# awsaf49/vip-cup-2022

Hardware: AMD Instinct MI355X
Metric: images/sec (200x200, full ensemble) (higher is better)
Workload: dtype f16; 1 GPU; ensemble8; precision=fast, distinct_images=5120, global_batch=256, parallelism=image-parallel dp1, one all-gather of scores, member_streams=3

## Files before the change

### include/vipcup_hip.h

```cpp
#ifndef VIPCUP_HIP_H
#define VIPCUP_HIP_H

#include <stddef.h>
#include <stdint.h>

#ifdef __cplusplus
extern "C" {
#endif

typedef enum vip_status {
    VIP_OK = 0,
    VIP_ERR_BAD_ARG = -1,
    VIP_ERR_ALIGNMENT = -2,
    VIP_ERR_UNSUPPORTED = -3,
    VIP_ERR_LAUNCH = -4,
    VIP_ERR_JPEG = -5,
    VIP_ERR_PNG = -6,
    VIP_ERR_WEBP = -7
} vip_status;

enum { VIP_ACT_NONE = 0, VIP_ACT_RELU = 1, VIP_ACT_SILU = 2, VIP_ACT_GELU = 3, VIP_ACT_SIGMOID = 4 };

int vip_version(void);
const char* vip_last_error(void);
// ... 34 lines not shown

int vip_ln_gemm_supported(int M, int K, int N, int act);
int vip_ln_gemm_bias_act_f16(const void* A, const float* ln_gamma, const float* ln_beta, float ln_eps, const void* W,
                             const float* bias, const void* residual, void* C, int M, int N, int K, int lda, int ldw,
                             int ldc, int ldr, int act_pre, int act_post, void* stream);

int vip_gemm_split_f16(const void* A, const void* W, const float* bias, void* C, int M, int N, int K, int lda,
                       int ldw, int act, void* stream);

int vip_gemm_split2_f16(const void* A, const void* W, const float* bias, void* C, int M, int N, int K, int ldw, int act,
                        void* stream);
int vip_gemm_split2_hilo_f16(const void* A, const void* W, const void* W_lo, const float* bias, void* C, int M, int N, int K, int ldw,
                             int act, void* stream);

int vip_mlp_fused_supported(int M, int C, int hidden, int act);
int vip_mlp_fused_plan(int M, int C, int hidden, int act, int* workgroups, int* tile_rows);
int vip_mlp_fused_f16(const void* x, const float* ln_gamma, const float* ln_beta, float ln_eps, const void* w1,
                      const float* b1, const void* w2, const float* b2, const void* residual, void* y, int M, int C,
                      int hidden, int ldx, int ldw1, int ldw2, int ldy, int ldr, int act, void* stream);

int vip_se_gate_f16(const void* x, const void* w1, const float* b1, const void* w2, const float* b2, void* gate,
                    int B, int HW, int C, int ldx, int Cr, int ldw1, int Cout, int ldw2, int act1, int act2,
                    int split, void* stream);
int vip_se_gate_hilo_f16(const void* x, const void* w1, const void* w1_lo, const float* b1, const void* w2, const float* b2, void* gate,
                         int B, int HW, int C, int ldx, int Cr, int ldw1, int Cout, int ldw2, int act1, int act2, int split,
                         void* stream);

int vip_dwconv2d_nhwc_f16(const void* x, const float* w, const float* bias, void* y,
                          int B, int H, int W, int C, int k, int stride, int pt, int pl,
                          int Ho, int Wo, int act, void* stream);

int vip_dwconv2d_pool_parts(int B, int H, int W, int C, int k, int stride, int Ho, int Wo);
long vip_dwconv2d_tile_plan(int B, int H, int W, int C, int k, int stride, int Ho, int Wo, int pooled, int* workgroups, int* geom);
int vip_dwconv2d_pool_nhwc_f16(const void* x, const float* w, const float* bias, void* y, float* partials, int parts,
                               int B, int H, int W, int C, int k, int stride, int pt, int pl, int Ho, int Wo, int act,
                               void* stream);
int vip_se_gate_pooled_f16(const float* partials, int parts, const void* w1, const float* b1, const void* w2,
                           const float* b2, void* gate, int B, int HW, int C, int Cr, int ldw1, int Cout, int ldw2,
                           int act1, int act2, int split, void* stream);

int vip_layernorm_f16(const void* x, const float* gamma, const float* beta, void* y,
                      int rows, int C, float eps, void* stream);

int vip_pool2d_nhwc_f16(const void* x, void* y, int B, int H, int W, int C, int ldx, int ldy,
                        int k, int stride, int pt, int pl, int Ho, int Wo, int mode, void* stream);

int vip_global_avgpool_f16(const void* x, void* y, int B, int HW, int C, int ldx, void* stream);

int vip_global_avgpool_split_f16(const void* x, void* y, int B, int HW, int C, int ldx, void* stream);

int vip_gap_dense_f32(const void* x, const float* W, const float* bias, float* out, int B, int HW, int C,
                      int ldx, int N, void* stream);

int vip_gap_ln_dense_f32(const void* x, const float* gamma, const float* beta, float eps, const float* W, const float* bias,
                         float* out, int B, int HW, int C, int ldx, int N, void* stream);

int vip_scale_add_act_f16(const void* x, const void* scale, const void* residual, void* y,
                          int B, int HW, int C, int act, void* stream);
int vip_scale_add_act2_f16(const void* x, const void* scale, const void* residual, void* y, void* y2,
                           int B, int HW, int C, int act, int act2, void* stream);
int vip_scale_add_act3_f16(const void* x, const void* scale, int scale_planes, const void* residual, void* y, void* y2,
                           int B, int HW, int C, int act, int act2, void* stream);

int vip_mul_f16(const void* a, const void* b, void* y, long rows, int C, int lda, int a_off, int ldb, int b_off,
                int ldy, int y_off, void* stream);

// ... 379 lines not shown
```

### vip-cup-2022_amd/_abi.py

```python
import ctypes as C
import os

import torch

_HERE = os.path.dirname(os.path.abspath(__file__))
LIB_PATH = os.environ.get("VIP_LIB_PATH") or os.path.join(_HERE, "libvipcup_hip.so")

_lib = None


class VipError(RuntimeError):
    pass


class ConvDesc(C.Structure):
    _fields_ = [(n, C.c_int) for n in (
        "B", "H", "W", "Cin", "Cout", "kh", "kw", "sh", "sw", "pt", "pl", "Ho", "Wo", "groups",
        "ldx", "cin_off", "ldy", "cout_off", "ldr", "res_off", "ldw", "act_pre", "act_post")]


class JpegDesc(C.Structure):
    _fields_ = [("width", C.c_int32), ("height", C.c_int32), ("ncomp", C.c_int32),
                ("hsamp", C.c_int32 * 3), ("vsamp", C.c_int32 * 3),
                ("blocks_w", C.c_int32 * 3), ("blocks_h", C.c_int32 * 3),
# ... 27 lines not shown

class Vp8EncParams(C.Structure):
    _fields_ = [("quality", C.c_int32), ("base_q", C.c_int32), ("y1", C.c_int32 * 2), ("y2", C.c_int32 * 2), ("uv", C.c_int32 * 2),
                ("filter_level", C.c_int32), ("flevel", C.c_int32), ("ilevel", C.c_int32), ("hev", C.c_int32), ("i4_bias", C.c_int32),
                ("reserved", C.c_int32), ("y1_inv", C.c_uint32 * 2), ("y2_inv", C.c_uint32 * 2), ("uv_inv", C.c_uint32 * 2)]


_vp, _i, _f, _sz = C.c_void_p, C.c_int, C.c_float, C.c_size_t

SIGNATURES = {
    "vip_version": (_i, []),
    "vip_last_error": (C.c_char_p, []),
    "vip_conv2d_nhwc_f16": (_i, [_vp, _vp, _vp, _vp, _vp, C.POINTER(ConvDesc), _vp]),
    "vip_conv2d_gated_nhwc_f16": (_i, [_vp, _vp, _vp, _vp, _vp, _vp, C.POINTER(ConvDesc), _vp]),
    "vip_conv2d_hilo_nhwc_f16": (_i, [_vp, _vp, _vp, _vp, _vp, _vp, C.POINTER(ConvDesc), _vp]),
    "vip_conv2d_out_gated_nhwc_f16": (_i, [_vp, _vp, _vp, _vp, _vp, _vp, _vp, C.POINTER(ConvDesc), _vp]),
    "vip_conv2d_out_gated_variant": (_i, [C.POINTER(ConvDesc), _i, C.c_char_p, _sz]),
    "vip_conv2d_out_gated2_nhwc_f16": (_i, [_vp, _vp, _vp, _vp, _vp, _vp, _vp, _vp, _i, C.POINTER(ConvDesc), _vp]),
    "vip_conv2d_out_gated2_variant": (_i, [C.POINTER(ConvDesc), _i, _i, C.c_char_p, _sz]),
    "vip_gemm_bias_act_f16": (_i, [_vp, _vp, _vp, _vp, _vp] + [_i] * 9 + [_vp]),
    "vip_ln_gemm_supported": (_i, [_i, _i, _i, _i]),
    "vip_ln_gemm_bias_act_f16": (_i, [_vp, _vp, _vp, _f] + [_vp] * 4 + [_i] * 9 + [_vp]),
    "vip_mlp_fused_supported": (_i, [_i, _i, _i, _i]),
    "vip_mlp_fused_plan": (_i, [_i] * 4 + [C.POINTER(_i)] * 2),
    "vip_mlp_fused_f16": (_i, [_vp, _vp, _vp, _f] + [_vp] * 6 + [_i] * 9 + [_vp]),
    "vip_se_gate_f16": (_i, [_vp] * 6 + [_i] * 11 + [_vp]),
    "vip_se_gate_hilo_f16": (_i, [_vp] * 7 + [_i] * 11 + [_vp]),
    "vip_gemm_split_f16": (_i, [_vp, _vp, _vp, _vp] + [_i] * 6 + [_vp]),
    "vip_gemm_split2_f16": (_i, [_vp, _vp, _vp, _vp] + [_i] * 5 + [_vp]),
    "vip_gemm_split2_hilo_f16": (_i, [_vp, _vp, _vp, _vp, _vp] + [_i] * 5 + [_vp]),
    "vip_dwconv2d_nhwc_f16": (_i, [_vp, _vp, _vp, _vp] + [_i] * 11 + [_vp]),
    "vip_dwconv2d_pool_parts": (_i, [_i] * 8),
    "vip_dwconv2d_tile_plan": (C.c_long, [_i] * 9 + [C.POINTER(_i)] * 2),
    "vip_dwconv2d_pool_nhwc_f16": (_i, [_vp, _vp, _vp, _vp, _vp] + [_i] * 12 + [_vp]),
    "vip_se_gate_pooled_f16": (_i, [_vp, _i] + [_vp] * 5 + [_i] * 10 + [_vp]),
    "vip_layernorm_f16": (_i, [_vp, _vp, _vp, _vp, _i, _i, _f, _vp]),
    "vip_pool2d_nhwc_f16": (_i, [_vp, _vp] + [_i] * 13 + [_vp]),
    "vip_global_avgpool_f16": (_i, [_vp, _vp, _i, _i, _i, _i, _vp]),
    "vip_global_avgpool_split_f16": (_i, [_vp, _vp, _i, _i, _i, _i, _vp]),
    "vip_gap_dense_f32": (_i, [_vp, _vp, _vp, _vp, _i, _i, _i, _i, _i, _vp]),
    "vip_experiments_built": (_i, []),
    "vip_gcvit_attn_block_supported": (_i, [_i, _i, _i]),
    "vip_gcvit_attn_block_f16": (_i, [_vp, _vp, _vp, _vp, _f, _vp, _i, _vp, _vp, _i, _vp, _vp, _vp] + [_i] * 6 + [_f, _vp]),
    "vip_mbconv_expand_dw_supported": (_i, [_i, _i, _i, _i]),
    "vip_mbconv_expand_dw_f16": (_i, [_vp] * 7 + [_i] * 14 + [_vp]),
    "vip_head_prob_f32": (_i, [_vp, _vp, _vp, _i, _i, _vp]),
    "vip_head_act_f32": (_i, [_vp, _vp, _i, _i, _i, _vp]),
    "vip_prob_to_score_f32": (_i, [_vp, _vp, _i, _i, _vp]),
    "vip_ensemble_mean_f32": (_i, [_vp, _vp, _i, _i, C.c_long, _vp]),
    "vip_gap_ln_dense_f32": (_i, [_vp, _vp, _vp, _f, _vp, _vp, _vp, _i, _i, _i, _i, _i, _vp]),
    "vip_scale_add_act_f16": (_i, [_vp, _vp, _vp, _vp, _i, _i, _i, _i, _vp]),
    "vip_scale_add_act2_f16": (_i, [_vp, _vp, _vp, _vp, _vp, _i, _i, _i, _i, _i, _vp]),
    "vip_scale_add_act3_f16": (_i, [_vp, _vp, _i, _vp, _vp, _vp, _i, _i, _i, _i, _i, _vp]),
    "vip_mul_f16": (_i, [_vp, _vp, _vp, C.c_long] + [_i] * 7 + [_vp]),
    "vip_radix_combine_f16": (_i, [_vp, _vp, _vp, _i, _i, _i, _i, _vp]),
    "vip_radix_combine2_f16": (_i, [_vp, _vp, _i, _vp, _i, _i, _i, _i, _vp]),
    "vip_window_attn_fwd_f16": (_i, [_vp, _vp, _vp, _vp] + [_i] * 7 + [_f, _vp]),
    "vip_mhsa_fwd_f16": (_i, [_vp, _vp, _i, _i, _i, _i, _f, _vp]),
    "vip_jpeg_probe_h": (_i, [_vp, _sz, _vp, _vp]),
    "vip_jpeg_entropy_decode_h": (_i, [_vp, _vp, _i, _vp, _vp, _sz, _vp, _i]),
    "vip_jpeg_idct_rgb_u8": (_i, [_vp, _vp, _i, _i, _vp, _vp, _i, _i, _vp]),
    "vip_jpeg_quality_tables_h": (_i, [_i, _vp, _vp]),
    "vip_jpeg_encode_layout_h": (_i, [_i, _i, _i, _i, _vp, _vp]),
    "vip_jpeg_fdct_quant_u8": (_i, [_vp, _vp, _i, _i, _vp, _vp, _i, _i, _vp]),
    "vip_resample_coeffs_h": (_i, [_i, _i, _i, _vp, _sz, _vp, _sz, _vp]),
    "vip_resample_tile_shape": (_i, [_vp, _vp, _vp]),
# ... 120 lines not shown
```

### vip-cup-2022_amd/csrc/common.hpp

```cpp
#pragma once
#include <hip/hip_runtime.h>
#include <stdint.h>
#include <stdio.h>
#include <stdarg.h>
#include "vipcup_hip.h"

#ifndef VIP_BUILD_EXPERIMENTS
#define VIP_BUILD_EXPERIMENTS 0
#endif

typedef _Float16 f16;
typedef _Float16 f16x8 __attribute__((ext_vector_type(8)));
typedef _Float16 f16x4 __attribute__((ext_vector_type(4)));
typedef _Float16 f16x2 __attribute__((ext_vector_type(2)));
typedef float f32x2 __attribute__((ext_vector_type(2)));
typedef float f32x4 __attribute__((ext_vector_type(4)));
typedef float f32x16 __attribute__((ext_vector_type(16)));

void vip_set_error(const char* fmt, ...);

#define VIP_REQUIRE(cond, code, ...)          \
    do {                                      \
        if (!(cond)) {                        \
            vip_set_error(__VA_ARGS__);       \
            return (code);                    \
        }                                     \
    } while (0)

static inline int vip_launch_status(const char* what) {
    hipError_t e = hipGetLastError();
    if (e != hipSuccess) {
        vip_set_error("%s: launch failed: %s", what, hipGetErrorString(e));
        return VIP_ERR_LAUNCH;
    }
    return VIP_OK;
}

int vip_dwconv_tiled(const void* x, const float* w, const float* bias, void* y, int B, int H, int W, int C, int k,
                     int pt, int pl, int Ho, int Wo, int act, hipStream_t s, float* partials = nullptr, int parts = 0);
int vip_dwconv_tiled_parts(int B, int H, int W, int C, int k, int Ho, int Wo);
long vip_dwconv_tiled_plan(int B, int H, int W, int C, int k, int Ho, int Wo, int pooled, int* workgroups, int* geom);
int vip_dwconv_tiled_h2(const void* x, const float* w, const float* bias, void* y, int B, int H, int W, int C, int k, int pt, int pl, int Ho,
                        int Wo, int act, int* status, hipStream_t s);
long vip_dwconv_tiled_plan_h2(int B, int H, int W, int C, int k, int Ho, int Wo, int* workgroups, int* geom);
int vip_window_attn_h2_mfma(const void* qkv, const void* q_global, const float* bias_table, void* out, int B, int Hp, int Wp, int C, int heads,
                            int ws, int nq, float scale, int* status, hipStream_t s);
int vip_mhsa_h2_mfma(const void* qkv, void* out, int B, int N, int D, int heads, float scale, int* status, hipStream_t s);
int vip_dwconv_mfma(const void* x, const float* w, const float* bias, void* y, int B, int H, int W, int C, int k,
                    int pt, int pl, int Ho, int Wo, int act, hipStream_t s);

int vip_gcvit_attn_block14(const void* x, const void* q_global, const float* ln_gamma, const float* ln_beta, float ln_eps, const void* wqkv,
                           int ldwq, const float* bqkv, const void* wproj, int ldwp, const float* bproj, const float* table, void* y,
                           int B, int Hp, int Wp, float scale, hipStream_t s);

__device__ __forceinline__ float vip_erf(float x) {
    const float ax = fabsf(x);
    const float t = __builtin_amdgcn_rcpf(fmaf(0.3275911f, ax, 1.0f));
    float p = fmaf(1.061405429f, t, -1.453152027f);
    p = fmaf(p, t, 1.421413741f);
    p = fmaf(p, t, -0.284496736f);
    p = fmaf(p, t, 0.254829592f);
    p = p * t;
    const float e = __builtin_amdgcn_exp2f(-ax * ax * 1.44269504088896f);
    return copysignf(fmaf(-p, e, 1.0f), x);
}
__device__ __forceinline__ float vip_sigmoid(float v) {
    return __builtin_amdgcn_rcpf(1.f + __builtin_amdgcn_exp2f(-v * 1.44269504088896f));
}

__device__ __forceinline__ f32x2 vip_gelu2(f32x2 x) {
    const f32x2 ax = {fabsf(x.x), fabsf(x.y)};
    f32x2 p = ax * 5.3829750e-06f + 4.8890636e-05f;
    p = p * ax + 3.8003575e-05f;
    p = p * ax + 3.2776263e-03f;
// ... 118 lines not shown
```

### vip-cup-2022_amd/csrc/dwconv.hip

```cpp
#include "common.hpp"

namespace {

static int VIP_DW_BLOCKS_PER_CU = 8;

typedef float f32x2 __attribute__((ext_vector_type(2)));


template <int T, int TW, int ACT, bool POOL>
__device__ __forceinline__ void dw_store(f32x2 (&acc)[T][TW][4], const float (&bv)[8], f16* __restrict__ y, int b, int oy0,
                                         int ox0, int Ho, int Wo, int C, int c0, f32x2 (&ps)[4]) {
#pragma unroll
    for (int oy = 0; oy < T; ++oy) {
        const int gy = oy0 + oy;
        if (gy >= Ho) break;
#pragma unroll
        for (int ox = 0; ox < TW; ++ox) {
            const int gx = ox0 + ox;
            if (gx >= Wo) break;
            U4H8 o;
#pragma unroll
            for (int e = 0; e < 4; ++e) {
                const f32x2 v = vip_act2<ACT>(acc[oy][ox][e] + (f32x2){bv[2 * e], bv[2 * e + 1]});
                o.e[2 * e] = (f16)v.x;
// ... 155 lines not shown
    float bv[8];
    {
        const float4 b0 = bias ? *reinterpret_cast<const float4*>(bias + c0) : make_float4(0.f, 0.f, 0.f, 0.f);
        const float4 b1 = bias ? *reinterpret_cast<const float4*>(bias + c0 + 4) : make_float4(0.f, 0.f, 0.f, 0.f);
        bv[0] = b0.x; bv[1] = b0.y; bv[2] = b0.z; bv[3] = b0.w;
        bv[4] = b1.x; bv[5] = b1.y; bv[6] = b1.z; bv[7] = b1.w;
    }
    f32x2 ps[4] = {{0.f, 0.f}, {0.f, 0.f}, {0.f, 0.f}, {0.f, 0.f}};
    switch (act) {
        case VIP_ACT_RELU: dw_store<T, TW, VIP_ACT_RELU, POOL>(acc, bv, y, b, oy0, ox0, Ho, Wo, C, c0, ps); break;
        case VIP_ACT_SILU: dw_store<T, TW, VIP_ACT_SILU, POOL>(acc, bv, y, b, oy0, ox0, Ho, Wo, C, c0, ps); break;
        case VIP_ACT_GELU: dw_store<T, TW, VIP_ACT_GELU, POOL>(acc, bv, y, b, oy0, ox0, Ho, Wo, C, c0, ps); break;
        case VIP_ACT_SIGMOID: dw_store<T, TW, VIP_ACT_SIGMOID, POOL>(acc, bv, y, b, oy0, ox0, Ho, Wo, C, c0, ps); break;
        default: dw_store<T, TW, VIP_ACT_NONE, POOL>(acc, bv, y, b, oy0, ox0, Ho, Wo, C, c0, ps); break;
    }
    if constexpr (POOL) {
        float* red = wlds + K * K * cb_chunks * 8;
        __syncthreads();
        if (lane_ok) {
            float* r = red + lt * (cb_chunks * 8) + lc * 8;
#pragma unroll
            for (int e = 0; e < 4; ++e) *reinterpret_cast<f32x2*>(r + 2 * e) = ps[e];
        }
        __syncthreads();
        if ((int)threadIdx.x < nch * 8) {
            float sum = 0.f;
            for (int t = 0; t < tiles_per_block; ++t) sum += red[t * (cb_chunks * 8) + threadIdx.x];
            partials[grp * C + c8_0 * 8 + threadIdx.x] = sum;
        }
    }
    }
}

template <int K, int T, int TW, bool WHOLE>
__global__ __launch_bounds__(256, 2) void dwconv_tile_h2_kernel(const char* __restrict__ x, const float* __restrict__ w,
                                                                const float* __restrict__ bias, char* __restrict__ y, int B, int H, int W,
                                                                int C, int pt, int pl, int Ho, int Wo, int act, int cb_chunks, int tiles_x,
                                                                int tiles_y, long n_tiles, long x_bytes, int* status) {
    constexpr int P = T + K - 1;
    constexpr int PW = TW + K - 1;
    extern __shared__ __attribute__((aligned(16))) float wlds[];

    const int c4_0 = blockIdx.y * cb_chunks;
    const int C4 = C >> 2;
    const int nch = min(cb_chunks, C4 - c4_0);
    for (int i = threadIdx.x; i < K * K * nch * 4; i += 256) {
        const int tap = i / (nch * 4), c = i - tap * (nch * 4);
        wlds[tap * (cb_chunks * 4) + c] = w[(long)tap * C + c4_0 * 4 + c];
    }
    __syncthreads();

    const int tiles_per_block = 256 / cb_chunks;
    const int lc = threadIdx.x % cb_chunks;
    const int lt = threadIdx.x / cb_chunks;
    if (!(lt < tiles_per_block && lc < nch)) return;
    const int c0 = (c4_0 + lc) * 4;
    const unsigned coff = (unsigned)((c0 >> 3) * 32 + ((c0 >> 2) & 1) * 8);
    const float* wl = wlds + lc * 4;
    const __amdgpu_buffer_rsrc_t rx = __builtin_amdgcn_make_buffer_rsrc((void*)x, 0, (unsigned)x_bytes, 0x00020000);

    const long n_groups = (n_tiles + tiles_per_block - 1) / tiles_per_block;
    long g_lo = 0, g_hi = n_groups, g_step = gridDim.x, g_first = blockIdx.x;
    if (gridDim.x >= 8) {
        const int xcd = blockIdx.x & 7;
        const long chunk = (n_groups + 7) / 8;
        g_lo = xcd * chunk;
// ... 178 lines not shown

template <int K, int T, int TW, bool WHOLE>
int launch_tile(const f16* x, const float* w, const float* bias, f16* y, int B, int H, int W, int C, int pt, int pl,
                int Ho, int Wo, int act, hipStream_t s, float* partials = nullptr, int parts = 0) {
    const DwTilePlan p = tile_plan<T, TW>(B, Ho, Wo, C, partials != nullptr);
    const size_t smem = (size_t)K * K * p.cb * 8 * sizeof(float);
    if (partials) {
        if (parts != p.gpi) {
            vip_set_error("vip_dwconv2d_pool_nhwc_f16: partials sized for %d rows per image, the kernel writes %d", parts, p.gpi);
            return VIP_ERR_BAD_ARG;
        }
        hipLaunchKernelGGL((dwconv_tile_kernel<K, T, TW, WHOLE, true>), dim3((unsigned)p.gx, (unsigned)p.gyc), dim3(256),
                           smem + (size_t)p.tiles_per_block * p.cb * 8 * sizeof(float), s, x, w, bias, y, B, H, W, C, pt, pl, Ho, Wo, act,
                           p.cb, p.tiles_x, p.tiles_y, p.n_tiles, 2L * B * H * W * C, partials, p.gpi);
        return vip_launch_status("vip_dwconv2d_pool_nhwc_f16(tile)");
    }
    hipLaunchKernelGGL((dwconv_tile_kernel<K, T, TW, WHOLE, false>), dim3((unsigned)p.gx, (unsigned)p.gyc), dim3(256), smem, s, x, w, bias,
                       y, B, H, W, C, pt, pl, Ho, Wo, act, p.cb, p.tiles_x, p.tiles_y, p.n_tiles, 2L * B * H * W * C, (float*)nullptr, 0);
    return vip_launch_status("vip_dwconv2d_nhwc_f16(tile)");
}

template <int T, int TW>
int tile_parts(int Ho, int Wo, int C) {
    const DwTilePlan p = tile_plan<T, TW>(1, Ho, Wo, C, true);
    if (p.tiles_x * p.tiles_y * 100 < p.gpi * p.tiles_per_block * 85) return 0;
    return p.gpi;
}

bool tile_shape_ok(int B, int H, int W, int C, int Ho, int Wo) {
    const long gx = ((long)B * ((Wo + 1) / 2) * ((Ho + 1) / 2) + 15) / 16;
    return !(gx >= (1L << 31) || 2L * B * H * W * C >= 0xFFFFFFF0L);
}

}

int vip_dwconv_tiled(const void* x, const float* w, const float* bias, void* y, int B, int H, int W, int C, int k,
                     int pt, int pl, int Ho, int Wo, int act, hipStream_t s, float* partials, int parts) {
    const f16* xi = (const f16*)x;
    const float* wi = w;
    f16* yo = (f16*)y;
    if (!tile_shape_ok(B, H, W, C, Ho, Wo)) return 1;
#define VIP_GO(KK, TT, WW, WH) return launch_tile<KK, TT, WW, WH>(xi, wi, bias, yo, B, H, W, C, pt, pl, Ho, Wo, act, s, partials, parts)
    if (k == 3) VIP_GO(3, 2, 4, true);
    if (k == 5) VIP_GO(5, 2, 2, false);
    if (k == 7) VIP_GO(7, 2, 4, false);
#undef VIP_GO
    return 1;
}

int vip_dwconv_tiled_h2(const void* x, const float* w, const float* bias, void* y, int B, int H, int W, int C, int k, int pt, int pl, int Ho,
                        int Wo, int act, int* status, hipStream_t s) {
    if (4L * B * H * W * C >= 0xFFFFFFE0L || C % 8 != 0) return 1;
#define VIP_GO(KK, TT, WW, WH) return launch_tile_h2<KK, TT, WW, WH>(x, w, bias, y, B, H, W, C, pt, pl, Ho, Wo, act, status, s)
    if (k == 3) VIP_GO(3, 2, 4, true);
    if (k == 5) VIP_GO(5, 2, 2, false);
    if (k == 7) VIP_GO(7, 2, 4, false);
#undef VIP_GO
    return 1;
}

int vip_dwconv_tiled_parts(int B, int H, int W, int C, int k, int Ho, int Wo) {
    if (!tile_shape_ok(B, H, W, C, Ho, Wo) || C % 8 != 0) return 0;
    if (k == 3) return tile_parts<2, 4>(Ho, Wo, C);
    if (k == 5) return tile_parts<2, 2>(Ho, Wo, C);
    if (k == 7) return tile_parts<2, 4>(Ho, Wo, C);
    return 0;
// ... 37 lines not shown
```

### vip-cup-2022_amd/csrc/pointwise.hip

```cpp
#include "common.hpp"

namespace {

__global__ __launch_bounds__(256) void pool2d_kernel(const f16* __restrict__ x, f16* __restrict__ y, int B, int H,
                                                     int W, int C8, int ldx, int ldy, int k, int stride, int pt,
                                                     int pl, int Ho, int Wo, int mode) {
    const long total = (long)B * Ho * Wo * C8;
    for (long idx = (long)blockIdx.x * 256 + threadIdx.x; idx < total; idx += (long)gridDim.x * 256) {
        const int c8 = (int)(idx % C8);
        long p = idx / C8;
        const int wo = (int)(p % Wo);
        p /= Wo;
        const int ho = (int)(p % Ho);
        const int b = (int)(p / Ho);
        float acc[8];
#pragma unroll
        for (int j = 0; j < 8; ++j) acc[j] = (mode == 0) ? -3.0e38f : 0.f;
        int cnt = 0;
        for (int r = 0; r < k; ++r) {
            const int hi = ho * stride - pt + r;
            for (int s = 0; s < k; ++s) {
                const int wi = wo * stride - pl + s;
                const bool ok = (unsigned)hi < (unsigned)H && (unsigned)wi < (unsigned)W;
                U4H8 v;
// ... 315 lines not shown
                VIP_ERR_BAD_ARG, "vip_dwconv2d_nhwc_f16: bad argument");
    VIP_REQUIRE(C % 8 == 0, VIP_ERR_ALIGNMENT, "vip_dwconv2d_nhwc_f16: C must be a multiple of 8");
    const int C8 = C / 8;
    hipStream_t s = (hipStream_t)stream;
    const f16* xi = (const f16*)x;
    const float* wi = w;
    f16* yo = (f16*)y;
    if (stride == 1) {
        const int sm = vip_dwconv_mfma(x, w, bias, y, B, H, W, C, k, pt, pl, Ho, Wo, act, s);
        if (sm != 1) return sm;
        const int st = vip_dwconv_tiled(x, w, bias, y, B, H, W, C, k, pt, pl, Ho, Wo, act, s);
        if (st != 1) return st;
    }
#define VIP_DW(KK, SS, TW)                                                                                        \
    {                                                                                                             \
        const long total = (long)B * Ho * ((Wo + TW - 1) / TW) * C8;                                              \
        hipLaunchKernelGGL((dwconv_kernel<KK, SS, TW>), dim3(grid_for(total)), dim3(256), 0, s, xi, wi, bias, yo, \
                           B, H, W, C8, pt, pl, Ho, Wo, act);                                                     \
    }
    if (k == 3 && stride == 1) VIP_DW(3, 1, 4)
    else if (k == 3 && stride == 2) VIP_DW(3, 2, 2)
    else if (k == 5 && stride == 1) VIP_DW(5, 1, 4)
    else if (k == 5 && stride == 2) VIP_DW(5, 2, 2)
    else if (k == 7 && stride == 1) VIP_DW(7, 1, 4)
    else {
        vip_set_error("vip_dwconv2d_nhwc_f16: unsupported k=%d stride=%d", k, stride);
        return VIP_ERR_UNSUPPORTED;
    }
#undef VIP_DW
    return vip_launch_status("vip_dwconv2d_nhwc_f16");
}

extern "C" int vip_dwconv2d_pool_parts(int B, int H, int W, int C, int k, int stride, int Ho, int Wo) {
    if (stride != 1 || B <= 0 || H <= 0 || W <= 0 || C <= 0 || Ho <= 0 || Wo <= 0) return 0;
    return vip_dwconv_tiled_parts(B, H, W, C, k, Ho, Wo);
}

extern "C" long vip_dwconv2d_tile_plan(int B, int H, int W, int C, int k, int stride, int Ho, int Wo, int pooled, int* workgroups, int* geom) {
    if (stride != 1 || B <= 0 || H <= 0 || W <= 0 || C <= 0 || Ho <= 0 || Wo <= 0) return 0;
    return vip_dwconv_tiled_plan(B, H, W, C, k, Ho, Wo, pooled, workgroups, geom);
}

extern "C" int vip_dwconv2d_pool_nhwc_f16(const void* x, const float* w, const float* bias, void* y, float* partials, int parts,
                                          int B, int H, int W, int C, int k, int stride, int pt, int pl, int Ho, int Wo, int act,
                                          void* stream) {
    VIP_REQUIRE(x && w && y && partials, VIP_ERR_BAD_ARG, "vip_dwconv2d_pool_nhwc_f16: null pointer");
    VIP_REQUIRE(B > 0 && H > 0 && W > 0 && C > 0 && Ho > 0 && Wo > 0 && pt >= 0 && pl >= 0 && (unsigned)act <= 4u,
                VIP_ERR_BAD_ARG, "vip_dwconv2d_pool_nhwc_f16: bad argument");
    VIP_REQUIRE(C % 8 == 0, VIP_ERR_ALIGNMENT, "vip_dwconv2d_pool_nhwc_f16: C must be a multiple of 8");
    VIP_REQUIRE(stride == 1 && parts > 0 && parts == vip_dwconv_tiled_parts(B, H, W, C, k, Ho, Wo), VIP_ERR_UNSUPPORTED,
                "vip_dwconv2d_pool_nhwc_f16: k=%d stride=%d parts=%d - ask vip_dwconv2d_pool_parts first", k, stride, parts);
    const int st = vip_dwconv_tiled(x, w, bias, y, B, H, W, C, k, pt, pl, Ho, Wo, act, (hipStream_t)stream, partials, parts);
    if (st == 1) {
        vip_set_error("vip_dwconv2d_pool_nhwc_f16: shape not handled by the tile kernel");
        return VIP_ERR_UNSUPPORTED;
    }
    return st;
}

namespace {
__global__ __launch_bounds__(256) void gap_dense_kernel(const f16* __restrict__ x, const float* __restrict__ Wt,
                                                        const float* __restrict__ bias, float* __restrict__ out,
                                                        int HW, int C, int ldx, int N) {
    __shared__ float pooled[4096];
    __shared__ float wsum[4];
    const int b = blockIdx.x;
    const f16* xb = x + (long)b * HW * ldx;
    const float inv = 1.f / (float)HW;
    for (int c8 = threadIdx.x; c8 < (C >> 3); c8 += 256) {
        float acc[8];
#pragma unroll
        for (int j = 0; j < 8; ++j) acc[j] = 0.f;
        for (int p = 0; p < HW; ++p) {
            U4H8 v;
            v.u = *reinterpret_cast<const uint4*>(xb + (long)p * ldx + c8 * 8);
#pragma unroll
            for (int j = 0; j < 8; ++j) acc[j] += (float)v.e[j];
        }
#pragma unroll
        for (int j = 0; j < 8; ++j) pooled[c8 * 8 + j] = acc[j] * inv;
    }
    __syncthreads();
    for (int n = 0; n < N; ++n) {
        float s = 0.f;
        for (int c = threadIdx.x; c < C; c += 256) s += pooled[c] * Wt[(long)n * C + c];
// ... 284 lines not shown
```

### vip-cup-2022_amd/ops.py

```python
import ctypes as C
import math
import os
from dataclasses import dataclass
from typing import Optional

import numpy as np
import torch

from . import _abi


def _env_flag(name: str, default: bool) -> bool:
    v = os.environ.get(name)
    return default if v is None else (v != "0" if default else v == "1")


def _env_int(name: str, default: int) -> int:
    return int(os.environ.get(name, default))


PRECISION = os.environ.get("VIP_PRECISION", "fast")
STRICT_GEMM = os.environ.get("VIP_STRICT_GEMM", "bf16x3")
_LN_GEMM = _env_flag("VIP_LN_GEMM", True)
_MLP_H2_FUSED = _env_flag("VIP_MLP_H2_FUSED", True)
# ... 833 lines not shown

def _dw_quad_major(w_khwc: torch.Tensor, k: int) -> torch.Tensor:
    key = (w_khwc.data_ptr(), w_khwc._version, tuple(w_khwc.shape))
    hit = _DW_QUAD.get(key)
    if hit is None:
        wq = torch.empty_like(w_khwc)
        _launch("vip_dw_filter_quad_major", _p(w_khwc), _p(wq), k, w_khwc.shape[-1])
        hit = _DW_QUAD[key] = (w_khwc, wq)
    return hit[1]


def dwconv2d(x, w_khwc: torch.Tensor, bias: Optional[torch.Tensor], k: int, stride=1, pad=(0, 0, 0, 0), act=None):
    kind = _kind(x, "dwconv2d.x")
    B, H, W, Cc = x.shape
    if not _dw_filter_ok(w_khwc, k, Cc):
        raise ValueError("dwconv2d: the filter must be a contiguous fp32 [k,k,C] tensor")
    pt, _, pl, _ = pad
    Ho, Wo = _out_hw(H, W, k, k, stride, stride, pad)
    out = torch.empty((B, Ho, Wo, Cc), dtype=x.dtype, device=x.device)
    if (kind == "h2" and _DW_H2_LDS and stride == 1 and k >= _DW_H2_LDS
            and _abi.lib().vip_dwconv2d_s1_supported_h2(B, H, W, Cc, k, Ho, Wo)):
        _launch("vip_dwconv2d_s1_h2", _p(x), _p(_dw_quad_major(w_khwc, k)), _p(bias), _p(out), B, H, W, Cc, k, pt, pl, Ho, Wo, _act(act),
                status=True)
    else:
        _launch_kind("dwconv2d_nhwc", kind, _p(x), _p(w_khwc), _p(bias), _p(out), B, H, W, Cc, k, stride, pt, pl, Ho, Wo, _act(act))
    return out


def dwconv2d_se(x, w_khwc: torch.Tensor, bias: Optional[torch.Tensor], k: int, stride, pad, act, fc1: ConvWeight, fc2: ConvWeight,
                act1, act2="sigmoid", split: bool = True):
    B, H, W, Cc = x.shape
    pt, _, pl, _ = pad
    Ho, Wo = _out_hw(H, W, k, k, stride, stride, pad)
    pooled = _DW_SE_FUSED and not _UNFUSED and stride == 1 and _se_chain_ok(fc1, fc2, Cc) and _dw_filter_ok(w_khwc, k, Cc)
    parts = 0
    if pooled and x.dtype == PACKED and _SE_H2_FUSED and _DW_H2_LDS and k >= _DW_H2_LDS and fc1.kind == fc2.kind == "h2":
        parts = _abi.lib().vip_dwconv2d_s1_pool_parts_h2(B, H, W, Cc, k, Ho, Wo)
    elif pooled and x.dtype == torch.float16 and not _CALIB and not _EXACT:
        parts = _abi.lib().vip_dwconv2d_pool_parts(B, H, W, Cc, k, stride, Ho, Wo)
    if parts <= 0:
        h = dwconv2d(x, w_khwc, bias, k, stride, pad, act=act)
        return h, se_gate(h, fc1, fc2, act1, act2, split=split)
    kind = _kind(x, "dwconv2d_se.x")
    h = torch.empty((B, Ho, Wo, Cc), dtype=x.dtype, device=x.device)
    partials = torch.empty((B, parts, Cc), dtype=torch.float32, device=x.device)
    if kind == "h2":
        _launch("vip_dwconv2d_s1_pool_h2", _p(x), _p(_dw_quad_major(w_khwc, k)), _p(bias), _p(h), _p(partials), parts, B, H, W, Cc, k,
                pt, pl, Ho, Wo, _act(act), status=True)
        gate = torch.empty((B, fc2.cout), dtype=PACKED, device=x.device)
        _launch("vip_se_gate_pooled_h2", _p(partials), parts, _p(fc1.w), _p(fc1.bias), 1.0 / fc1.h2_scale, _p(fc2.w), _p(fc2.bias),
                1.0 / fc2.h2_scale, _p(gate), B, Ho * Wo, Cc, fc1.cout, fc1.ldw, fc2.cout, fc2.ldw, _act(act1), _act(act2), status=True)
    else:
        _launch("vip_dwconv2d_pool_nhwc_f16", _p(x), _p(w_khwc), _p(bias), _p(h), _p(partials), parts, B, H, W, Cc, k, stride, pt, pl,
                Ho, Wo, _act(act))
        gate = torch.empty((B, 2, fc2.cout) if split else (B, fc2.cout), dtype=torch.float16, device=x.device)
        _launch("vip_se_gate_pooled_f16", _p(partials), parts, _p(fc1.w), _p(fc1.bias), _p(fc2.w), _p(fc2.bias), _p(gate), B, Ho * Wo,
                Cc, fc1.cout, fc1.ldw, fc2.cout, fc2.ldw, _act(act1), _act(act2), int(split))
    return h, gate


def mbconv_expand_dw(x, cw: ConvWeight, w_khwc: torch.Tensor, dw_bias: Optional[torch.Tensor], k: int, stride: int, pad, act=None):
    B, H, W, ldx = x.shape
    ok = (not _UNFUSED and x.dtype == torch.float16 and mbconv_fused() and _pointwise(cw) and ldx == cw.cin
          and w_khwc.shape == (k, k, cw.cout) and _abi.lib().vip_mbconv_expand_dw_supported(cw.cin, cw.cout, k, stride))
    if not ok:
        return dwconv2d(conv2d(x, cw, act=act), w_khwc, dw_bias, k, stride, pad, act=act)
    _chk16(x, "mbconv_expand_dw.x")
    Ho, Wo = _out_hw(H, W, k, k, stride, stride, pad)
    out = torch.empty((B, Ho, Wo, cw.cout), dtype=torch.float16, device=x.device)
# ... 378 lines not shown
```

Measured before the change: 4914 images/sec.

## Add stride-2 tiled depthwise conv kernel with fused SE pooling partials

Adds a stride-2 variant of the tiled depthwise-conv kernel that also writes per-tile channel sums for squeeze-excite pooling, plus a planner for it. dwconv2d_se now takes the fused dwconv+pool path for stride-2 layers (k=3 or 5, fp16), where it previously ran the depthwise conv and then a separate SE gate that re-read the activation. This saves one full pass over the stride-2 activation and one launch per such block. In exchange there is a new kernel with its own register and LDS pressure and reduction barriers, and it is only taken for the plain f16 path, not the packed h2 path.

```diff
diff --git a/include/vipcup_hip.h b/include/vipcup_hip.h
--- a/include/vipcup_hip.h
+++ b/include/vipcup_hip.h
@@ -90,6 +90,7 @@
 
 int vip_dwconv2d_pool_parts(int B, int H, int W, int C, int k, int stride, int Ho, int Wo);
 long vip_dwconv2d_tile_plan(int B, int H, int W, int C, int k, int stride, int Ho, int Wo, int pooled, int* workgroups, int* geom);
+long vip_dwconv2d_tile_plan_s2(int B, int H, int W, int C, int k, int Ho, int Wo, int* workgroups, int* geom);
 int vip_dwconv2d_pool_nhwc_f16(const void* x, const float* w, const float* bias, void* y, float* partials, int parts,
                                int B, int H, int W, int C, int k, int stride, int pt, int pl, int Ho, int Wo, int act,
                                void* stream);
diff --git a/vip-cup-2022_amd/_abi.py b/vip-cup-2022_amd/_abi.py
--- a/vip-cup-2022_amd/_abi.py
+++ b/vip-cup-2022_amd/_abi.py
@@ -83,6 +83,7 @@
     "vip_dwconv2d_nhwc_f16": (_i, [_vp, _vp, _vp, _vp] + [_i] * 11 + [_vp]),
     "vip_dwconv2d_pool_parts": (_i, [_i] * 8),
     "vip_dwconv2d_tile_plan": (C.c_long, [_i] * 9 + [C.POINTER(_i)] * 2),
+    "vip_dwconv2d_tile_plan_s2": (C.c_long, [_i] * 7 + [C.POINTER(_i)] * 2),
     "vip_dwconv2d_pool_nhwc_f16": (_i, [_vp, _vp, _vp, _vp, _vp] + [_i] * 12 + [_vp]),
     "vip_se_gate_pooled_f16": (_i, [_vp, _i] + [_vp] * 5 + [_i] * 10 + [_vp]),
     "vip_layernorm_f16": (_i, [_vp, _vp, _vp, _vp, _i, _i, _f, _vp]),
diff --git a/vip-cup-2022_amd/csrc/common.hpp b/vip-cup-2022_amd/csrc/common.hpp
--- a/vip-cup-2022_amd/csrc/common.hpp
+++ b/vip-cup-2022_amd/csrc/common.hpp
@@ -40,6 +40,10 @@
                      int pt, int pl, int Ho, int Wo, int act, hipStream_t s, float* partials = nullptr, int parts = 0);
 int vip_dwconv_tiled_parts(int B, int H, int W, int C, int k, int Ho, int Wo);
 long vip_dwconv_tiled_plan(int B, int H, int W, int C, int k, int Ho, int Wo, int pooled, int* workgroups, int* geom);
+int vip_dwconv_tiled_s2(const void* x, const float* w, const float* bias, void* y, int B, int H, int W, int C, int k, int pt, int pl,
+                        int Ho, int Wo, int act, hipStream_t s, float* partials, int parts);
+int vip_dwconv_tiled_s2_parts(int B, int H, int W, int C, int k, int Ho, int Wo);
+long vip_dwconv_tiled_s2_plan(int B, int H, int W, int C, int k, int Ho, int Wo, int* workgroups, int* geom);
 int vip_dwconv_tiled_h2(const void* x, const float* w, const float* bias, void* y, int B, int H, int W, int C, int k, int pt, int pl, int Ho,
                         int Wo, int act, int* status, hipStream_t s);
 long vip_dwconv_tiled_plan_h2(int B, int H, int W, int C, int k, int Ho, int Wo, int* workgroups, int* geom);
diff --git a/vip-cup-2022_amd/csrc/dwconv.hip b/vip-cup-2022_amd/csrc/dwconv.hip
--- a/vip-cup-2022_amd/csrc/dwconv.hip
+++ b/vip-cup-2022_amd/csrc/dwconv.hip
@@ -211,6 +211,154 @@
     }
 }
 
+template <int K, int T, int TW, int DEPTH, int BLOCKS>
+__global__ __launch_bounds__(256, BLOCKS) void dwconv_tile_s2_kernel(const f16* __restrict__ x, const float* __restrict__ w,
+                                                                const float* __restrict__ bias, f16* __restrict__ y, int B, int H, int W,
+                                                                int C, int pt, int pl, int Ho, int Wo, int act, int cb_chunks, int tiles_x,
+                                                                int tiles_y, long x_bytes, float* __restrict__ partials, int gpi) {
+    constexpr int P = (T - 1) * 2 + K;
+    constexpr int PW = (TW - 1) * 2 + K;
+    constexpr int CS = K * K * 8 + 4;
+    static_assert(DEPTH >= 1 && DEPTH <= P, "rows requested ahead of the one being multiplied");
+    extern __shared__ __attribute__((aligned(16))) float wlds[];
+
+    const int c8_0 = blockIdx.y * cb_chunks;
+    const int C8 = C >> 3;
+    const int nch = min(cb_chunks, C8 - c8_0);
+    for (int i = threadIdx.x; i < K * K * nch * 8; i += 256) {
+        const int tap = i / (nch * 8), c = i - tap * (nch * 8);
+        wlds[(c >> 3) * CS + tap * 8 + (c & 7)] = w[(long)tap * C + c8_0 * 8 + c];
+    }
+    __syncthreads();
+
+    const int tiles_per_block = 256 / cb_chunks;
+    int lc = threadIdx.x % cb_chunks;
+    const int lt = threadIdx.x / cb_chunks;
+    const bool lane_ok = lt < tiles_per_block && lc < nch;
+    if (lc >= nch) lc = nch - 1;
+    const int c0 = (c8_0 + lc) * 8;
+    const float* wl = wlds + lc * CS;
+    const __amdgpu_buffer_rsrc_t rx = __builtin_amdgcn_make_buffer_rsrc((void*)x, 0, (unsigned)x_bytes, 0x00020000);
+
+    const long n_groups = (long)B * gpi;
+    long g_lo = 0, g_hi = n_groups, g_step = gridDim.x, g_first = blockIdx.x;
+    if (gridDim.x >= 8) {
+        const int xcd = blockIdx.x & 7;
+        const long chunk = (n_groups + 7) / 8;
+        g_lo = xcd * chunk;
+        g_hi = min(n_groups, g_lo + chunk);
+        g_step = (gridDim.x + 7 - xcd) >> 3;
+        g_first = g_lo + (blockIdx.x >> 3);
+    }
+    for (long grp = g_first; grp < g_hi; grp += g_step) {
+        const int b = (int)(grp / gpi);
+        const int ti = (int)(grp - (long)b * gpi) * tiles_per_block + lt;
+        const bool work = lane_ok && ti < tiles_x * tiles_y;
+        const int tx = work ? ti % tiles_x : 0;
+        const int ty = work ? ti / tiles_x : tiles_y;
+        const int oy0 = ty * T, ox0 = tx * TW;
+
+        f32x2 acc[T][TW][4];
+#pragma unroll
+        for (int i = 0; i < T; ++i)
+#pragma unroll
+            for (int j = 0; j < TW; ++j)
+#pragma unroll
+                for (int q = 0; q < 4; ++q) acc[i][j][q] = (f32x2){0.f, 0.f};
+
+        const unsigned row_bytes = (unsigned)W * (unsigned)C * 2u;
+        bool col_ok[PW];
+#pragma unroll
+        for (int q = 0; q < PW; ++q) col_ok[q] = (unsigned)(ox0 * 2 - pl + q) < (unsigned)W;
+        int row_gy = oy0 * 2 - pt;
+        unsigned row_off = (unsigned)((((long)b * H * W) * C + c0) * 2) + (unsigned)(row_gy * W + ox0 * 2 - pl) * ((unsigned)C * 2u);
+        asm volatile("" : "+v"(row_off));
+        auto load_row = [&](uint4 (&raw)[PW]) {
+            const bool row_ok = (unsigned)row_gy < (unsigned)H;
+#pragma unroll
+            for (int q = 0; q < PW; ++q) {
+                const unsigned off = (row_ok & col_ok[q]) ? row_off + (unsigned)q * ((unsigned)C * 2u) : 0xFFFFFFF0u;
+                raw[q] = __builtin_bit_cast(uint4, __builtin_amdgcn_raw_buffer_load_b128(rx, off, 0, 0));
+            }
+            ++row_gy;
+            row_off += row_bytes;
+            __builtin_amdgcn_sched_barrier(0);
+        };
+        auto mac_row = [&](int iy, const uint4 (&rawrow)[PW]) {
+            f32x2 xr[PW][4];
+#pragma unroll
+            for (int q = 0; q < PW; ++q) {
+                U4H8 v;
+                v.u = rawrow[q];
+#pragma unroll
+                for (int e = 0; e < 4; ++e) {
+                    xr[q][e][0] = (float)v.e[2 * e];
+                    xr[q][e][1] = (float)v.e[2 * e + 1];
+                }
+            }
+#pragma unroll
+            for (int oy = 0; oy < T; ++oy) {
+                const int r = iy - 2 * oy;
+                if (r < 0 || r >= K) continue;
+#pragma unroll
+                for (int s = 0; s < K; ++s) {
+                    const float4 w0 = *reinterpret_cast<const float4*>(wl + (r * K + s) * 8);
+                    const float4 w1 = *reinterpret_cast<const float4*>(wl + (r * K + s) * 8 + 4);
+                    const f32x2 wv[4] = {{w0.x, w0.y}, {w0.z, w0.w}, {w1.x, w1.y}, {w1.z, w1.w}};
+#pragma unroll
+                    for (int ox = 0; ox < TW; ++ox)
+#pragma unroll
+                        for (int e = 0; e < 4; ++e) acc[oy][ox][e] = xr[2 * ox + s][e] * wv[e] + acc[oy][ox][e];
+                }
+            }
+#pragma unroll
+            for (int oy = 0; oy < T; ++oy)
+#pragma unroll
+                for (int ox = 0; ox < TW; ++ox)
+#pragma unroll
+                    for (int e = 0; e < 4; ++e) asm volatile("" : "+v"(acc[oy][ox][e]));
+            __builtin_amdgcn_sched_barrier(0);
+        };
+        uint4 raw[P][PW];
+#pragma unroll
+        for (int iy = 0; iy < DEPTH; ++iy) load_row(raw[iy]);
+#pragma unroll
+        for (int iy = 0; iy < P; ++iy) {
+            if (iy + DEPTH < P) load_row(raw[iy + DEPTH]);
+            mac_row(iy, raw[iy]);
+        }
+
+        float bv[8];
+        {
+            const float4 b0 = bias ? *reinterpret_cast<const float4*>(bias + c0) : make_float4(0.f, 0.f, 0.f, 0.f);
+            const float4 b1 = bias ? *reinterpret_cast<const float4*>(bias + c0 + 4) : make_float4(0.f, 0.f, 0.f, 0.f);
+            bv[0] = b0.x; bv[1] = b0.y; bv[2] = b0.z; bv[3] = b0.w;
+            bv[4] = b1.x; bv[5] = b1.y; bv[6] = b1.z; bv[7] = b1.w;
+        }
+        f32x2 ps[4] = {{0.f, 0.f}, {0.f, 0.f}, {0.f, 0.f}, {0.f, 0.f}};
+        switch (act) {
+            case VIP_ACT_RELU: dw_store<T, TW, VIP_ACT_RELU, true>(acc, bv, y, b, oy0, ox0, Ho, Wo, C, c0, ps); break;
+            case VIP_ACT_SILU: dw_store<T, TW, VIP_ACT_SILU, true>(acc, bv, y, b, oy0, ox0, Ho, Wo, C, c0, ps); break;
+            case VIP_ACT_GELU: dw_store<T, TW, VIP_ACT_GELU, true>(acc, bv, y, b, oy0, ox0, Ho, Wo, C, c0, ps); break;
+            case VIP_ACT_SIGMOID: dw_store<T, TW, VIP_ACT_SIGMOID, true>(acc, bv, y, b, oy0, ox0, Ho, Wo, C, c0, ps); break;
+            default: dw_store<T, TW, VIP_ACT_NONE, true>(acc, bv, y, b, oy0, ox0, Ho, Wo, C, c0, ps); break;
+        }
+        float* red = wlds + cb_chunks * CS;
+        __syncthreads();
+        if (lane_ok) {
+            float* r = red + lt * (cb_chunks * 8) + lc * 8;
+#pragma unroll
+            for (int e = 0; e < 4; ++e) *reinterpret_cast<f32x2*>(r + 2 * e) = ps[e];
+        }
+        __syncthreads();
+        if ((int)threadIdx.x < nch * 8) {
+            float sum = 0.f;
+            for (int t = 0; t < tiles_per_block; ++t) sum += red[t * (cb_chunks * 8) + threadIdx.x];
+            partials[grp * C + c8_0 * 8 + threadIdx.x] = sum;
+        }
+    }
+}
+
 template <int K, int T, int TW, bool WHOLE>
 __global__ __launch_bounds__(256, 2) void dwconv_tile_h2_kernel(const char* __restrict__ x, const float* __restrict__ w,
                                                                 const float* __restrict__ bias, char* __restrict__ y, int B, int H, int W,
@@ -455,6 +603,80 @@
     return !(gx >= (1L << 31) || 2L * B * H * W * C >= 0xFFFFFFF0L);
 }
 
+template <int T, int TW>
+DwTilePlan tile_plan_s2(int B, int Ho, int Wo, int C) {
+    DwTilePlan p;
+    const int C8 = C / 8;
+    p.tiles_x = (Wo + TW - 1) / TW;
+    p.tiles_y = (Ho + T - 1) / T;
+    const int tiles = p.tiles_x * p.tiles_y;
+    p.n_tiles = (long)B * tiles;
+    long best = -1;
+    p.cb = 1;
+    for (int cb = C8 < 32 ? C8 : 32; cb >= (C8 < 8 ? C8 : 8); --cb) {
+        const int tpb = 256 / cb;
+        const long lanes = 256L * ((C8 + cb - 1) / cb) * ((tiles + tpb - 1) / tpb);
+        if (best < 0 || lanes < best) {
+            best = lanes;
+            p.cb = cb;
+        }
+    }
+    p.tiles_per_block = 256 / p.cb;
+    p.gyc = (C8 + p.cb - 1) / p.cb;
+    p.gpi = (tiles + p.tiles_per_block - 1) / p.tiles_per_block;
+    p.groups = (long)B * p.gpi;
+    p.gx_cap = (256L * VIP_DW_BLOCKS_PER_CU + p.gyc - 1) / p.gyc;
+    p.gx = p.groups > p.gx_cap ? p.gx_cap : p.groups;
+    return p;
+}
+
+bool plan_s2(int B, int H, int W, int C, int k, int Ho, int Wo, DwTilePlan& p) {
+    if (B <= 0 || H <= 0 || W <= 0 || C <= 0 || C % 8 != 0 || Ho <= 0 || Wo <= 0 || 2L * B * H * W * C >= 0xFFFFFFF0L) return false;
+    if (k == 3) p = tile_plan_s2<2, 2>(B, Ho, Wo, C);
+    else if (k == 5) p = tile_plan_s2<2, 2>(B, Ho, Wo, C);
+    else return false;
+    return p.groups < (1L << 31);
+}
+
+template <int K, int T, int TW, int DEPTH, int BLOCKS>
+int launch_tile_s2(const DwTilePlan& p, const f16* x, const float* w, const float* bias, f16* y, int B, int H, int W, int C, int pt, int pl,
+                   int Ho, int Wo, int act, hipStream_t s, float* partials) {
+    const size_t smem = ((size_t)p.cb * (K * K * 8 + 4) + (size_t)p.tiles_per_block * p.cb * 8) * sizeof(float);
+    hipLaunchKernelGGL((dwconv_tile_s2_kernel<K, T, TW, DEPTH, BLOCKS>), dim3((unsigned)p.gx, (unsigned)p.gyc), dim3(256), smem, s, x, w, bias, y, B,
+                       H, W, C, pt, pl, Ho, Wo, act, p.cb, p.tiles_x, p.tiles_y, 2L * B * H * W * C, partials, p.gpi);
+    return vip_launch_status("vip_dwconv2d_pool_nhwc_f16(tile, stride 2)");
+}
+
+}
+
+int vip_dwconv_tiled_s2(const void* x, const float* w, const float* bias, void* y, int B, int H, int W, int C, int k, int pt, int pl,
+                        int Ho, int Wo, int act, hipStream_t s, float* partials, int parts) {
+    DwTilePlan p;
+    if (!partials || !plan_s2(B, H, W, C, k, Ho, Wo, p)) return 1;
+    if (parts != p.gpi) {
+        vip_set_error("vip_dwconv2d_pool_nhwc_f16: partials sized for %d rows per image, the kernel writes %d", parts, p.gpi);
+        return VIP_ERR_BAD_ARG;
+    }
+    if (k == 3) return launch_tile_s2<3, 2, 2, 2, 3>(p, (const f16*)x, w, bias, (f16*)y, B, H, W, C, pt, pl, Ho, Wo, act, s, partials);
+    return launch_tile_s2<5, 2, 2, 2, 2>(p, (const f16*)x, w, bias, (f16*)y, B, H, W, C, pt, pl, Ho, Wo, act, s, partials);
+}
+
+int vip_dwconv_tiled_s2_parts(int B, int H, int W, int C, int k, int Ho, int Wo) {
+    DwTilePlan p;
+    return plan_s2(B, H, W, C, k, Ho, Wo, p) ? p.gpi : 0;
+}
+
+long vip_dwconv_tiled_s2_plan(int B, int H, int W, int C, int k, int Ho, int Wo, int* workgroups, int* geom) {
+    DwTilePlan p;
+    if (!plan_s2(B, H, W, C, k, Ho, Wo, p)) return 0;
+    if (workgroups) *workgroups = (int)p.gx;
+    if (geom) {
+        geom[0] = p.cb;
+        geom[1] = p.tiles_per_block;
+        geom[2] = p.gyc;
+        geom[3] = (int)p.gx_cap;
+    }
+    return p.groups;
 }
 
 int vip_dwconv_tiled(const void* x, const float* w, const float* bias, void* y, int B, int H, int W, int C, int k,
diff --git a/vip-cup-2022_amd/csrc/pointwise.hip b/vip-cup-2022_amd/csrc/pointwise.hip
--- a/vip-cup-2022_amd/csrc/pointwise.hip
+++ b/vip-cup-2022_amd/csrc/pointwise.hip
@@ -371,13 +371,18 @@
 }
 
 extern "C" int vip_dwconv2d_pool_parts(int B, int H, int W, int C, int k, int stride, int Ho, int Wo) {
-    if (stride != 1 || B <= 0 || H <= 0 || W <= 0 || C <= 0 || Ho <= 0 || Wo <= 0) return 0;
-    return vip_dwconv_tiled_parts(B, H, W, C, k, Ho, Wo);
+    if (B <= 0 || H <= 0 || W <= 0 || C <= 0 || Ho <= 0 || Wo <= 0) return 0;
+    if (stride == 2) return vip_dwconv_tiled_s2_parts(B, H, W, C, k, Ho, Wo);
+    return stride == 1 ? vip_dwconv_tiled_parts(B, H, W, C, k, Ho, Wo) : 0;
 }
 
 extern "C" long vip_dwconv2d_tile_plan(int B, int H, int W, int C, int k, int stride, int Ho, int Wo, int pooled, int* workgroups, int* geom) {
     if (stride != 1 || B <= 0 || H <= 0 || W <= 0 || C <= 0 || Ho <= 0 || Wo <= 0) return 0;
     return vip_dwconv_tiled_plan(B, H, W, C, k, Ho, Wo, pooled, workgroups, geom);
+}
+
+extern "C" long vip_dwconv2d_tile_plan_s2(int B, int H, int W, int C, int k, int Ho, int Wo, int* workgroups, int* geom) {
+    return vip_dwconv_tiled_s2_plan(B, H, W, C, k, Ho, Wo, workgroups, geom);
 }
 
 extern "C" int vip_dwconv2d_pool_nhwc_f16(const void* x, const float* w, const float* bias, void* y, float* partials, int parts,
@@ -387,9 +392,10 @@
     VIP_REQUIRE(B > 0 && H > 0 && W > 0 && C > 0 && Ho > 0 && Wo > 0 && pt >= 0 && pl >= 0 && (unsigned)act <= 4u,
                 VIP_ERR_BAD_ARG, "vip_dwconv2d_pool_nhwc_f16: bad argument");
     VIP_REQUIRE(C % 8 == 0, VIP_ERR_ALIGNMENT, "vip_dwconv2d_pool_nhwc_f16: C must be a multiple of 8");
-    VIP_REQUIRE(stride == 1 && parts > 0 && parts == vip_dwconv_tiled_parts(B, H, W, C, k, Ho, Wo), VIP_ERR_UNSUPPORTED,
+    VIP_REQUIRE(parts > 0 && parts == vip_dwconv2d_pool_parts(B, H, W, C, k, stride, Ho, Wo), VIP_ERR_UNSUPPORTED,
                 "vip_dwconv2d_pool_nhwc_f16: k=%d stride=%d parts=%d - ask vip_dwconv2d_pool_parts first", k, stride, parts);
-    const int st = vip_dwconv_tiled(x, w, bias, y, B, H, W, C, k, pt, pl, Ho, Wo, act, (hipStream_t)stream, partials, parts);
+    const int st = stride == 2 ? vip_dwconv_tiled_s2(x, w, bias, y, B, H, W, C, k, pt, pl, Ho, Wo, act, (hipStream_t)stream, partials, parts)
+                               : vip_dwconv_tiled(x, w, bias, y, B, H, W, C, k, pt, pl, Ho, Wo, act, (hipStream_t)stream, partials, parts);
     if (st == 1) {
         vip_set_error("vip_dwconv2d_pool_nhwc_f16: shape not handled by the tile kernel");
         return VIP_ERR_UNSUPPORTED;
diff --git a/vip-cup-2022_amd/ops.py b/vip-cup-2022_amd/ops.py
--- a/vip-cup-2022_amd/ops.py
+++ b/vip-cup-2022_amd/ops.py
@@ -889,9 +889,9 @@
     B, H, W, Cc = x.shape
     pt, _, pl, _ = pad
     Ho, Wo = _out_hw(H, W, k, k, stride, stride, pad)
-    pooled = _DW_SE_FUSED and not _UNFUSED and stride == 1 and _se_chain_ok(fc1, fc2, Cc) and _dw_filter_ok(w_khwc, k, Cc)
+    pooled = _DW_SE_FUSED and not _UNFUSED and stride in (1, 2) and _se_chain_ok(fc1, fc2, Cc) and _dw_filter_ok(w_khwc, k, Cc)
     parts = 0
-    if pooled and x.dtype == PACKED and _SE_H2_FUSED and _DW_H2_LDS and k >= _DW_H2_LDS and fc1.kind == fc2.kind == "h2":
+    if pooled and stride == 1 and x.dtype == PACKED and _SE_H2_FUSED and _DW_H2_LDS and k >= _DW_H2_LDS and fc1.kind == fc2.kind == "h2":
         parts = _abi.lib().vip_dwconv2d_s1_pool_parts_h2(B, H, W, Cc, k, Ho, Wo)
     elif pooled and x.dtype == torch.float16 and not _CALIB and not _EXACT:
         parts = _abi.lib().vip_dwconv2d_pool_parts(B, H, W, Cc, k, stride, Ho, Wo)
```

Result: no change. 4944 images/sec (median of 6 runs) (+0.6%).
